# rikuu/Gap2Seq

Hardware: AMD Instinct MI355X
Metric: gaps filled/sec (whole node), k=31 synthetic 3 Mbp DBG (higher is better)
Workload: dtype u32

## Files before the change

### gap2seq_amd/csrc/d3_device.h

```cpp
#pragma once
#include <hip/hip_runtime_api.h>
#include <stdint.h>

#include "d2_device.h"
#include "fill_device.h"

#define G2S_D3_BLOCK_VARS 16u
#define G2S_RAND_BLOCK 4096u
#define G2S_RAND_WINDOW 160u
#define G2S_D3_TABLE_BUDGET (8u << 20)

#define G2S_D3_UNHANDLED 0x1u
#define G2S_D3_BUDGET 0x2u
#define G2S_D3_ANOMALY 0x4u

namespace g2s {

struct D3Gap {
  uint64_t arena_off;
  int32_t skip_thr;
  uint16_t lmf;
  uint8_t kind;
  uint8_t pad;
};
// ... 32 lines not shown
static_assert(sizeof(D3Var) == 64 && sizeof(D3Trace) == 32, "record layouts");

struct D3Summary {
  uint32_t status, unhandled, n_var, anomalies;
  unsigned long long host_items, host_segs, host_rnd;
  uint32_t handoff_waves, tiles;
  uint64_t table_entries, block_entries;
  uint64_t draws_min, draws_spread, draws_total;
  uint64_t xA, sA, xB, sB, xD, sD, segs, fill_bytes;
  uint32_t seg_gaps, filled;
  uint32_t rand_state[31];
  uint32_t trace_waves;
  uint32_t big_gaps;
  uint32_t traced_gaps;
  uint32_t spec_gaps;
};
static_assert(sizeof(D3Summary) <= 512, "the lap stamps live at byte 512 of the summary's slot");

struct RandTables {
  const uint32_t* hi = nullptr;
  const uint32_t* mid = nullptr;
  const uint32_t* lane = nullptr;
};
void rand_tables_host(uint32_t* hi , uint32_t* mid , uint32_t* lane );

struct D3Work {
  uint32_t* ginfo = nullptr;
  uint32_t* dmin = nullptr;
  uint32_t* dspread = nullptr;
  uint32_t* base = nullptr;
// ... 29 lines not shown
  int32_t k, skip_confident, all_paths, unique_paths;
  uint64_t max_states;
  uint64_t arena_base;
  uint32_t n;
  uint32_t has_skip;
  uint32_t seg_cap;
  uint32_t map_cap;
  uint32_t group_size;
  uint64_t sub_region;
  uint32_t laps;
  uint32_t self_clean;
  uint32_t base0, R0, d_in;
  const unsigned long long* d2_done;
  uint32_t d2_wgs;
  uint32_t restart;
};

hipError_t launch_rand_fill(hipStream_t st, uint32_t* rnd_all, const RandTables& rt, const D3Summary* sum_dev, uint64_t capacity,
                            uint64_t first_value = 0);

hipError_t launch_d3_sharded_classes(hipStream_t st, const D3Params& P, const D3Work& W, const GapOut* outs, const D3Gap* dgaps,
                                     bool summary_is_clean);
hipError_t launch_d3_sharded_tables(hipStream_t st, const D3Params& P, const D3Work& W, const GapOut* outs, const SubRec* sub,
                                    uint32_t* rnd_all, uint64_t rnd_capacity, uint32_t* group_fn );
hipError_t launch_d3_sharded_trace(hipStream_t st, const D3Params& P, const D3Work& W, const GapOut* outs, const SubRec* sub,
                                   const char* lastch_up, const char* lastch_dn, uint32_t* rnd_all, uint64_t rnd_capacity,
                                   void* results, char* arena, const D3Side& side, void* summary_host,
                                   hipEvent_t ev_d2 = nullptr );

hipError_t launch_rand_window(hipStream_t st, uint32_t* rnd_all, const uint32_t* link);
// ... 15 lines not shown
```

### gap2seq_amd/csrc/d3_device.hip

```cpp
#include "sync_debug.h"
#include <hip/hip_runtime.h>
#include <hip/hip_ext.h>

#include <algorithm>
#include <cstdlib>
#include <mutex>
#include <set>

#include "../../include/g2s.h"
#include "d3_device.h"
#include "envcache.hpp"

namespace {

using g2s::D3Gap;
using g2s::D3Params;
using g2s::D3Summary;
using g2s::D3Work;

__device__ __forceinline__ uint32_t uni(uint32_t x) { return (uint32_t)__builtin_amdgcn_readfirstlane((int)x); }

#define GI_CLASS(x) ((x) & 3u)
#define GI_FILLED 0x4u
#define GI_SKIPPED 0x8u
#define GI_BAD 0x10u
#define GI_MEM 0x20u
#define GI_PHASE_D 0x40u
#define D3_TILE 256u
#define GI_HOST 0x80u

__device__ __forceinline__ void stamp(const D3Work& W, int slot) {
  ((unsigned long long*)((char*)W.sum + 512))[slot] = wall_clock64();
}

__device__ __forceinline__ const SubRec* sub_of(const D3Params& P, const SubRec* sub, uint32_t i) {
  return sub + (uint64_t)(i / P.group_size) * P.sub_region;
}

__device__ __forceinline__ int gap_count(const GapOut& go, const D3Params& P, bool phase_d) {
  if (phase_d && !P.skip_confident && P.all_paths) return go.count_s;
  return go.c_count;
}

// ... 491 lines not shown
    const int d0 = (int)(s.depth_len & 0xFFFFu);
    if (d0 > len) break;
    if (s.flags & G2S_SUB_SOURCE) return 1 + len - d0;
    if (d0 == 0) break;
    const int nb = seg_nparents(s.par01, s.par23);
    const uint32_t at = (uint32_t)(1 + len - d0);
    if (nb == 0 || (nb > 1 && !(s.flags & G2S_SEG_ORDERED)) || (uint64_t)at >= avail || at >= nwin) break;
    const uint32_t rv = nb > 1 ? lwin[at] >> 1 : 0u;
    i = (int)seg_parent(s.par01, s.par23, nb == 1 ? 0 : pick_parent(rv, nb));
    if (i >= nsegs) break;
  }
  *bad = true;
  return 1;
}

#define D3_TAB_SEGS 512u
__global__ __launch_bounds__(256) void g2s_d3_tables(const D3Params P, const D3Work W, const SubRec* __restrict__ sub,
                                                     const uint32_t* __restrict__ rnd , uint64_t capacity) {
  __shared__ SegLite lseg[D3_TAB_SEGS];
  extern __shared__ __attribute__((aligned(16))) uint32_t lwin[];
  const uint32_t win_cap = P.map_cap + D3_TILE;
  const D3Summary* S = W.sum;
  const bool st0 = blockIdx.x == 0 && threadIdx.x == 0;
  if (st0) stamp(W, 3);
  const uint32_t status = S->status, tiles = S->tiles;
  const uint32_t tid = threadIdx.x;
  if (status) return;
  if (st0) stamp(W, 4);
  bool bad_any = false;
  for (uint32_t tile = blockIdx.x; tile < tiles; tile += gridDim.x) {
    const uint32_t v = W.tile_var[tile];
    const g2s::D3Var vd = W.vdesc[v];
    const uint32_t ns = vd.ns;
    const uint32_t d0 = (tile - vd.tile0) * D3_TILE, d = d0 + tid;
    const uint64_t at0 = (uint64_t)vd.base + d0;
    const bool mine = d <= vd.R;
    const uint32_t want = min(win_cap, min(vd.R - d0, D3_TILE - 1u) + vd.dmin + vd.dspread + 1u);
    if (st0) stamp(W, 5);
    __syncthreads();
    {
      const SegW* gs = (const SegW*)(sub + vd.sub_at);
      for (uint32_t q = tid; q < ns && q < D3_TAB_SEGS; q += 256u) {
        SegLite l;
        l.depth_len = gs[q].depth_len; l.par01 = gs[q].par01; l.par23 = gs[q].par23; l.flags = gs[q].flags;
        lseg[q] = l;
      }
      for (uint32_t x = tid; x < want; x += 256u) lwin[x] = at0 + x < capacity ? rnd[at0 + x] : 0u;
    }
    __syncthreads();
    if (st0) stamp(W, 6);
    if (mine) {
      bool bad = false;
      const uint64_t at = at0 + tid;
      const uint32_t nw = want > tid ? want - tid : 0u;
      const uint64_t av = capacity > at ? capacity - at : 0ull;
      const int draws = ns > D3_TAB_SEGS
                            ? d3_walk_count(vd.n_len, vd.len0, vd.len1, vd.start_seg, vd.start_t, (int)ns, (const SegW*)(sub + vd.sub_at), lwin + tid, nw, av, &bad)
                            : d3_walk_count_lite(vd.n_len, vd.len0, vd.len1, vd.start_seg, (int)ns, lseg, lwin + tid, nw, av, &bad);
      const int dev = draws - (int)vd.dmin;
      if (dev < 0 || dev > (int)vd.dspread) bad = true;
      W.tab[(uint64_t)vd.toff + d] = bad ? (uint16_t)0 : (uint16_t)dev;
      bad_any |= bad;
    }
  }
  if (bad_any) atomicAdd(&W.sum->anomalies, 1u);
  if (st0) stamp(W, 7);
  if (P.laps && tid == 0) {
    unsigned long long* laps = (unsigned long long*)((char*)W.sum + 512);
    if (blockIdx.x < tiles) atomicMax(&laps[32], wall_clock64());
    atomicMax(&laps[33], wall_clock64());
  }
}

__device__ __forceinline__ void d3_blocks_body(const D3Work& W, uint64_t first, uint64_t stride) {
  const D3Summary* S = W.sum;
  const uint32_t V = S->n_var;
  const uint32_t NB = (V + G2S_D3_BLOCK_VARS - 1u) / G2S_D3_BLOCK_VARS;
  const uint64_t TB = S->block_entries;
  for (uint64_t e = first; e < TB; e += stride) {
    uint32_t lo = 0, hi = NB;
    while (hi - lo > 1u) { const uint32_t mid = (lo + hi) >> 1; if ((uint64_t)W.blk_toff[mid] <= e) lo = mid; else hi = mid; }
    const uint32_t b = lo;
    uint32_t d = (uint32_t)(e - W.blk_toff[b]);
    const uint32_t v1 = min(V, (b + 1u) * G2S_D3_BLOCK_VARS);
    for (uint32_t v = b * G2S_D3_BLOCK_VARS; v < v1; v++) d += W.tab[(uint64_t)W.var_toff[v] + d];
    W.btab[e] = d;
  }
}
// ... 183 lines not shown
  (void)d3_classify_body(P, W, outs, dgaps, blockIdx.x * 256u + threadIdx.x, gridDim.x * 256u, nullptr, nullptr, nullptr, nullptr, red, false);
  (void)d3_handoff_body<true>(P, W, outs, sub, rnd, capacity, side, blockIdx.x * 256u + (threadIdx.x & ~63u), nullptr, nullptr, nullptr, nullptr);
  if ((threadIdx.x & 63u) == 0u) {
    asm volatile("s_waitcnt vmcnt(0)" ::: "memory");
    const unsigned int done = atomicAdd(&S->handoff_waves, 1u) + 1u;
    if (done == gridDim.x * 4u) {
      const unsigned long long items = atomicAdd(&S->host_items, 0ull);
      const uint32_t anomalies = atomicAdd(&S->anomalies, 0u), unhandled = atomicAdd(&S->unhandled, 0u);
      S->status = unhandled ? G2S_D3_UNHANDLED : 0u;
      __hip_atomic_store(side.count, (items & 0x7FFFFFFFFFFFFFFFull) | ((unsigned long long)((anomalies || unhandled) ? 1u : 0u) << 63),
                         __ATOMIC_RELEASE, __HIP_MEMORY_SCOPE_SYSTEM);
    }
  }
}
#define D3_BACK_TAB 24576u
__global__ __launch_bounds__(1024) void g2s_d3_back(const D3Params P, const D3Work W, const GapOut* __restrict__ outs,
                                                    const SubRec* __restrict__ sub, const uint32_t* __restrict__ Wd, uint64_t capacity,
                                                    const g2s::D3Side side) {
  __shared__ uint32_t total_dev;
  __shared__ unsigned long long lcur[3];
  if (threadIdx.x < 3u) lcur[threadIdx.x] = 0ull;
  __shared__ uint16_t ltab[D3_BACK_TAB];
  __shared__ uint32_t ltoff[1025], ldvar[1025];
  D3Summary* S = W.sum;
  if (threadIdx.x == 0) stamp(W, 8);
  const uint32_t status = S->status, V = S->n_var;
  const uint64_t T = S->table_entries;
  if (status) {
    if (threadIdx.x == 0) __hip_atomic_store(side.count, 1ull << 63, __ATOMIC_RELEASE, __HIP_MEMORY_SCOPE_SYSTEM);
    return;
  }
  const bool in_lds = T <= (uint64_t)D3_BACK_TAB && V <= 1024u;
  if (in_lds) {
    for (uint32_t e = threadIdx.x; e < (uint32_t)T; e += 1024u) ltab[e] = W.tab[e];
    if (threadIdx.x <= V) ltoff[threadIdx.x] = W.var_toff[threadIdx.x];
    __syncthreads();
    if (threadIdx.x == 0) {
      stamp(W, 9);
      uint32_t d = 0;
      for (uint32_t v = 0; v < V; v++) { ldvar[v] = d; d += ltab[ltoff[v] + d]; }
      ldvar[V] = d;
      total_dev = d;
    }
    __syncthreads();
    if (threadIdx.x <= V) W.dvar[threadIdx.x] = ldvar[threadIdx.x];
    const uint64_t total = S->draws_min + total_dev;
    if (threadIdx.x == 0) S->draws_total = total;
    if (threadIdx.x < 31u) {
      const uint32_t w = Wd[total + threadIdx.x];
      S->rand_state[threadIdx.x] = w;
      if (W.link) W.link[threadIdx.x] = w;
    }
  } else {
    d3_blocks_body(W, threadIdx.x, 1024u);
    __threadfence();
    __syncthreads();
    d3_chain_body(W, Wd, &total_dev);
    __threadfence();
    __syncthreads();
  }
  if (threadIdx.x == 0) stamp(W, 10);
  for (uint32_t i0 = (threadIdx.x >> 6) * 64u; i0 < P.n; i0 += 1024u)
    (void)d3_handoff_body<false>(P, W, outs, sub, Wd + 31, capacity, side, i0, in_lds ? ldvar : nullptr, in_lds ? ltab : nullptr,
                          in_lds ? ltoff : nullptr, lcur);
  __syncthreads();
  if (threadIdx.x == 0) {
    stamp(W, 11);
    const unsigned long long items = lcur[0];
    S->host_items = items; S->host_segs = lcur[1]; S->host_rnd = lcur[2];
    const uint32_t anomalies = atomicAdd(&S->anomalies, 0u);
    __hip_atomic_store(side.count, (items & 0x7FFFFFFFFFFFFFFFull) | ((unsigned long long)(anomalies ? 1u : 0u) << 63), __ATOMIC_RELEASE,
                       __HIP_MEMORY_SCOPE_SYSTEM);
    stamp(W, 12);
  }
}

template <int NW>
__global__ __launch_bounds__(64 * NW) void g2s_d3_trace(const D3Params P, const D3Work W, GapOut* __restrict__ outs,
                                                   const SubRec* __restrict__ sub, const char* __restrict__ chu,
                                                   const char* __restrict__ chd, const uint32_t* __restrict__ rnd,
                                                   uint64_t capacity, g2s_result* __restrict__ results,
                                                   char* __restrict__ arena, uint32_t* __restrict__ summary_host,
                                                   const g2s::D3Side side, uint32_t* __restrict__ clean_words ) {
  extern __shared__ __attribute__((aligned(16))) uint32_t lds[];
  D3Summary* S = W.sum;
  const uint32_t i = blockIdx.x;
  constexpr int NT = 64 * NW;
  const int tid = (int)threadIdx.x, lane = tid & 63;
  const bool w0 = tid < 64;
// ... 34 lines not shown
  if ((go.dflags & G2S_DEVA_D2_PENDING) && !(go.dflags & (G2S_DEVA_RUNS | G2S_DEVA_D2_FAILED)) && !P.skip_confident) {
    uint32_t v = go.dflags;
    for (uint32_t spin = 0; spin < (1u << 22) && !(v & (G2S_DEVA_RUNS | G2S_DEVA_D2_FAILED)); spin++) {
      __builtin_amdgcn_s_sleep(8);
      v = uni(__hip_atomic_load(&outs[i].dflags, __ATOMIC_ACQUIRE, __HIP_MEMORY_SCOPE_AGENT));
    }
    __builtin_amdgcn_fence(__ATOMIC_ACQUIRE, "agent");
    go.dflags = v;
    go.sub_vertices = uni(__hip_atomic_load(&outs[i].sub_vertices, __ATOMIC_RELAXED, __HIP_MEMORY_SCOPE_AGENT));
    go.sub_edges = uni(__hip_atomic_load(&outs[i].sub_edges, __ATOMIC_RELAXED, __HIP_MEMORY_SCOPE_AGENT));
    if (!(v & (G2S_DEVA_RUNS | G2S_DEVA_D2_FAILED))) d2_lost = true;
  }
  if ((go.dflags & G2S_DEVA_D2_PENDING) && (go.dflags & G2S_DEVA_D2_FAILED) && !(td.gi & GI_HOST) && (td.gi & GI_PHASE_D)) d2_lost = true;
  uint32_t gsp_all = 0, gsp_sent = 0;
  auto leave = [&](uint32_t fill_len) {
    if (!w0) return;
    uint32_t last = 0;
    if (lane == 0) {
      if (P.laps) {
        const unsigned long long tk4 = wall_clock64();
        atomicMax(&laps[14], tk1 ? tk1 - tk0 : 0ull); atomicMax(&laps[15], tk2 ? tk2 - tk1 : 0ull);
        atomicMax(&laps[16], tk3 ? tk3 - tk2 : 0ull); atomicMax(&laps[17], ((tk4 - tk0) << 24) | ((td.gi & GI_HOST) ? 1ull << 23 : 0ull) | (unsigned long long)(i & 0x7FFFFFu)); atomicMax(&laps[18], tk4);
        atomicMax(&laps[19], ((tk2 ? tk2 - tk1 : 0ull) << 32) | (hops << 16) | (tkm ? tkm - tk1 : 0ull));
        if ((P.laps >> 4) == i + 1u) { laps[26] = tk0; laps[27] = tk1; laps[28] = tkm; laps[29] = tk2; laps[30] = tk3; laps[31] = tk4; }
      }
      const uint32_t c = i & 63u, n = gridDim.x;
      const unsigned long long before = atomicAdd(&W.fill_bytes[c * 16u], (unsigned long long)fill_len | (1ull << 40));
      if (gsp_all) atomicAdd(&W.fill_bytes[c * 16u + 1u], (unsigned long long)gsp_all | ((unsigned long long)gsp_sent << 32));
      if ((uint32_t)(before >> 40) + 1u == (n + 63u - c) / 64u) last = atomicAdd(&S->trace_waves, 1u) + 1u == min(n, 64u) ? 1u : 0u;
    }
// ... 2 lines not shown
    if (P.d2_done && lane == 0)
      for (uint32_t spin = 0; spin < (1u << 22) && __hip_atomic_load(P.d2_done, __ATOMIC_ACQUIRE, __HIP_MEMORY_SCOPE_AGENT) < (unsigned long long)P.d2_wgs; spin++)
        __builtin_amdgcn_s_sleep(8);
    uint32_t* src = (uint32_t*)S;
    if (P.laps && lane == 0) laps[24] = wall_clock64();
    static_assert(sizeof(D3Summary) <= 512, "two words a lane");
    const uint32_t s0 = __hip_atomic_load(src + lane, __ATOMIC_RELAXED, __HIP_MEMORY_SCOPE_AGENT);
    const uint32_t s1 = __hip_atomic_load(src + 64 + lane, __ATOMIC_RELAXED, __HIP_MEMORY_SCOPE_AGENT);
    const unsigned long long* cl = (const unsigned long long*)(src + 256 + 32 * lane);
    const unsigned long long c0 = __hip_atomic_load(cl, __ATOMIC_RELAXED, __HIP_MEMORY_SCOPE_AGENT);
    const unsigned long long c1 = __hip_atomic_load(cl + 1, __ATOMIC_RELAXED, __HIP_MEMORY_SCOPE_AGENT);
    summary_host[lane] = s0;
    summary_host[64 + lane] = s1;
    ((unsigned long long*)(summary_host + 256 + 32 * lane))[0] = c0;
    ((unsigned long long*)(summary_host + 256 + 32 * lane))[1] = c1;
    if (P.self_clean) {
      src[lane] = 0u; src[64 + lane] = 0u;
      ((unsigned long long*)(src + 256 + 32 * lane))[0] = 0ull;
      ((unsigned long long*)(src + 256 + 32 * lane))[1] = 0ull;
    }
    if (P.self_clean && clean_words && lane < 32) clean_words[lane] = 0u;
    if (P.laps && lane == 0) { asm volatile("s_waitcnt vmcnt(0)" ::: "memory"); laps[25] = wall_clock64(); }
  };
  if (status) { leave(0u); return; }
  if (d2_lost) {
    if (tid == 0) { atomicAdd(&S->anomalies, 1u); arena[td.arena_off + td.lmf] = '\0'; }
    asm volatile("s_waitcnt vmcnt(0)" ::: "memory");
    leave(0u);
    return;
  }
// ... 470 lines not shown
  if (P.n == 0) return hipSuccess;
  hipError_t e = summary_is_clean ? hipSuccess : hipMemsetAsync(W.sum, 0, 1024 + 64 * 128, st);
  if (e != hipSuccess) return e;
  hipLaunchKernelGGL(g2s_d3_classify, dim3((P.n + 255u) / 256u), dim3(256), 0, st, P, W, outs, dgaps);
  launch_scan(st, P, W, outs);
  return hipGetLastError();
}
hipError_t launch_d3_sharded_tables(hipStream_t st, const D3Params& P, const D3Work& W, const GapOut* outs, const SubRec* sub,
                                    uint32_t* rnd_all, uint64_t rnd_capacity, uint32_t* group_fn) {
  if (P.n == 0) return hipSuccess;
  launch_scan(st, P, W, outs);
  const uint32_t tgrid = std::min(8192u, std::max(128u, P.n / 2u));
  const size_t win = ((size_t)P.map_cap + 256) * 4;
  hipError_t e = hipFuncSetAttribute((const void*)g2s_d3_tables, hipFuncAttributeMaxDynamicSharedMemorySize, (int)win);
  if (e != hipSuccess) return e;
  hipLaunchKernelGGL(g2s_d3_tables, dim3(tgrid), dim3(256), win, st, P, W, sub, rnd_all + 31, rnd_capacity);
  hipLaunchKernelGGL(g2s_d3_blocks, dim3(256), dim3(256), 0, st, W);
  hipLaunchKernelGGL(g2s_d3_groupfn, dim3(std::min(256u, (P.R0 + 256u) / 256u)), dim3(256), 0, st, W, P.R0, group_fn);
  return hipGetLastError();
}
hipError_t launch_d3_sharded_trace(hipStream_t st, const D3Params& P, const D3Work& W, const GapOut* outs, const SubRec* sub,
                                   const char* lastch_up, const char* lastch_dn, uint32_t* rnd_all, uint64_t rnd_capacity,
                                   void* results, char* arena, const D3Side& side, void* summary_host, hipEvent_t ev_d2) {
  if (P.n == 0) return hipSuccess;
  hipLaunchKernelGGL(g2s_d3_chain, dim3(1), dim3(1024), 0, st, W, rnd_all, P.base0, P.d_in);
  if (ev_d2) { const hipError_t e2 = hipStreamWaitEvent(st, ev_d2, 0); if (e2 != hipSuccess) return e2; }
  hipLaunchKernelGGL(g2s_d3_handoff, dim3((P.n + 63u) / 64u), dim3(64), 0, st, P, W, outs, sub, rnd_all + 31, rnd_capacity, side);
  const size_t lds = (size_t)P.seg_cap * (sizeof(SegRec) + 16) + (size_t)P.map_cap * 8 + 16;
  hipError_t e = hipFuncSetAttribute((const void*)g2s_d3_trace<1>, hipFuncAttributeMaxDynamicSharedMemorySize, (int)lds);
  if (e != hipSuccess) return e;
  hipLaunchKernelGGL(g2s_d3_trace<1>, dim3(P.n), dim3(64), lds, st, P, W, const_cast<GapOut*>(outs), sub, lastch_up, lastch_dn, rnd_all + 31, rnd_capacity,
// ... 10 lines not shown
  (void)gaps;
  (void)rt;
  static_assert(sizeof(D3Summary) <= 1024, "summary slot");
  hipError_t e = summary_is_clean ? hipSuccess : hipMemsetAsync(W.sum, 0, 1024 + 64 * 128, st);
  if (e != hipSuccess) return e;
  const bool short_list = P.n <= D3_FRONT_GAPS;
  if (P.restart) {
    if (ev_d2) { e = hipStreamWaitEvent(st, ev_d2, 0); if (e != hipSuccess) return e; }
    hipLaunchKernelGGL(g2s_d3_restart, dim3((P.n + 255u) / 256u), dim3(256), 0, st, P, W, outs, dgaps, sub, rnd_all + 31, rnd_capacity, side);
  } else if (short_list) hipLaunchKernelGGL(g2s_d3_front, dim3(1), dim3(1024), 0, st, P, W, outs, dgaps);
  else {
    hipLaunchKernelGGL(g2s_d3_classify, dim3((P.n + 255u) / 256u), dim3(256), 0, st, P, W, outs, dgaps);
    launch_scan(st, P, W, outs);
  }
  const uint32_t tgrid = std::min(8192u, std::max(128u, P.n / 2u));
  const size_t win = ((size_t)P.map_cap + 256) * 4;
  if (!P.restart) {
    e = hipFuncSetAttribute((const void*)g2s_d3_tables, hipFuncAttributeMaxDynamicSharedMemorySize, (int)win);
    if (e != hipSuccess) return e;
    hipLaunchKernelGGL(g2s_d3_tables, dim3(tgrid), dim3(256), win, st, P, W, sub, rnd_all + 31, rnd_capacity);
  }
  if (ev_d2 && short_list && !P.restart) { e = hipStreamWaitEvent(st, ev_d2, 0); if (e != hipSuccess) return e; }
  if (P.restart) (void)ev_chain;
  else if (short_list) {
    hipLaunchKernelGGL(g2s_d3_back, dim3(1), dim3(1024), 0, st, P, W, outs, sub, rnd_all, rnd_capacity, side);
    if (ev_chain) { e = hipEventRecord(ev_chain, st); if (e != hipSuccess) return e; }
  } else {
    hipLaunchKernelGGL(g2s_d3_blocks, dim3(256), dim3(256), 0, st, W);
    hipLaunchKernelGGL(g2s_d3_chain, dim3(1), dim3(1024), 0, st, W, rnd_all, 0u, 0u);
    if (ev_chain) { e = hipEventRecord(ev_chain, st); if (e != hipSuccess) return e; }
    if (ev_d2) { e = hipStreamWaitEvent(st, ev_d2, 0); if (e != hipSuccess) return e; }
    hipLaunchKernelGGL(g2s_d3_handoff, dim3((P.n + 63u) / 64u), dim3(64), 0, st, P, W, outs, sub, rnd_all + 31, rnd_capacity, side);
  }
  const size_t lds = (size_t)P.seg_cap * (sizeof(SegRec) + 16) + (size_t)P.map_cap * 8 + 16;
  const char* waves_s = GENV("G2S_TRACE_WAVES");
  const int waves_env = waves_s ? atoi(waves_s) : 0;
  const bool four = waves_env ? waves_env == 4 : P.n <= 768u;
  e = hipFuncSetAttribute(four ? (const void*)g2s_d3_trace<4> : (const void*)g2s_d3_trace<1>, hipFuncAttributeMaxDynamicSharedMemorySize, (int)lds);
  if (e != hipSuccess) return e;
  if (ev_stop != nullptr) {
// ... 19 lines not shown
```

### gap2seq_amd/csrc/g2s_api.hip

```cpp
#include <hip/hip_runtime.h>
#include <cstdarg>
#include <sys/prctl.h>
#include <pthread.h>
#include <sched.h>
#include <time.h>

#include <algorithm>
#include <atomic>
#include <chrono>
#include <cstdio>
#include <cstdlib>
#include <condition_variable>
#include <cstring>
#include <functional>
#include <mutex>
#include <string>
#include <thread>
#include <vector>

#include "../../include/g2s.h"
#include "../../include/g2s_test.h"
#include "envcache.hpp"
#include "d2_device.h"
#include "d3_device.h"
// ... 681 lines not shown
  int team_sessions = 1;
  int peer_asked_for = -1;
  bool self_cleaned = false;
  std::vector<uint32_t> host_order;
  size_t side_dirty = SIZE_MAX;
  size_t side_layout_n = 0;
  uint32_t timed_seq = 0;
  std::chrono::steady_clock::time_point lap_fill_queued, lap_d3_queued, lap_handed, lap_finished, lap_synced, lap_end;
  bool laps_valid = false;
  int resident_strikes = 0;
  int segw_quiet = 0;
  hipEvent_t ev_segw = nullptr;
  g2s_session* twins[G2S_MAX_IN_FLIGHT - 1] = {};
  DevBuf d_link;
  hipEvent_t ev_chain = nullptr;
  void* d3_pending = nullptr;
  struct InFlight { g2s_batch* b = nullptr; g2s_session* on = nullptr; g2s_result* results = nullptr; char* arena = nullptr; size_t cap = 0;
                    const g2s_gap* gaps = nullptr; size_t n = 0; double ms_prepare = 0;
                    bool d3_queued = false;
                    bool chained = false; };
  InFlight inflight[G2S_MAX_IN_FLIGHT];
  int n_inflight = 0;
  int internal_calls = 0;
  uint64_t begun = 0;
  g2s_batch* share_batch = nullptr;
  int share_step = 0;
  bool share_timed = false, share_two = false;
  uint32_t share_win[G2S_RAND_WINDOW];
  bool resident_off = false;
  uint32_t seed0 = 0;
// ... 2304 lines not shown
  bool discard = false;
  D3Side side_h;
  D3Work W;
  D3Summary* hsum = nullptr;
  hipEvent_t d3_begin = nullptr;
  g2s_result* results = nullptr;
  char* arena = nullptr;
  std::chrono::steady_clock::time_point t_enter, t_launched;
  bool sharded = false;
  D3Params P;
  D3Side side_dev;
  void* res_dev = nullptr;
  char* arena_dev = nullptr;
  const D3Gap* dgaps_dev = nullptr;
  void* summary_dev = nullptr;
  uint32_t* group_fn = nullptr;
  uint32_t* group_fn_dev = nullptr;
  size_t rnd_cap = 0;
};
static int resident_d3_launch(g2s_session* s, const ResidentList& L, bool timed, bool rand_launched, g2s_result* results, char* arena,
                              bool no_spin, bool sharded = false ,
                              g2s_session* chain_from = nullptr ) {
  const size_t n = L.n;
  const Graph& g = *s->graph->g;
  const FillParams fp = fill_params_of(s);
  const auto t_enter = std::chrono::steady_clock::now();
  if (n > 20480 || L.dmax > 12000 || rand_capacity(L.rnd_cap) >= (1ull << 31)) return 1;
  if (hipSetDevice(s->device) != hipSuccess) return fail(G2S_ERR_NO_DEVICE, "cannot select device");
  D3Summary* hsum = (D3Summary*)((char*)L.pin->p + n * sizeof(D3Gap) + 16 - (n * sizeof(D3Gap)) % 16);
  const size_t rnd_cap = rand_capacity(L.rnd_cap);
  HIP_TRY_S(s->d_d3.ensure(d3_work_bytes((uint32_t)n)));
  D3Side side, side_h;
  {
    side_h.cap_items = n;
    const bool deep = L.dmax >= 2500;
    side_h.cap_segs = deep ? std::min<uint64_t>((uint64_t)n * 4096u, 4ull << 20) + 65536u : std::max<uint64_t>((uint64_t)n * 16u, 65536u);
    const size_t side_rnd = std::max(rnd_cap, rand_capacity(L.rnd_sum));
// ... 61 lines not shown
  memset(&P, 0, sizeof P);
  P.k = fp.k; P.skip_confident = fp.skip_confident ? 1 : 0; P.all_paths = fp.all_paths ? 1 : 0; P.unique_paths = fp.unique_paths ? 1 : 0;
  P.max_states = (uint64_t)std::max<int64_t>(s->params.max_mem, 1 << 16) / 64;
  P.n = (uint32_t)n;
  P.has_skip = L.has_skip ? 1u : 0u;
  P.arena_base = 0;
  P.group_size = (uint32_t)std::max<size_t>(L.group_size, 1);
  P.sub_region = L.sub_region;
  P.laps = GENV("G2S_DEBUG") ? (1u | (GENV("G2S_DEBUG_GAP") ? ((uint32_t)atoi(GENV("G2S_DEBUG_GAP")) + 1u) << 4 : 0u)) : 0u;
  const bool self_clean = L.groups.size() == 1 && L.outs_dev == (const GapOut*)s->d_outs.p && !P.laps && !sharded;
  P.self_clean = self_clean ? 1u : 0u;
  if (W.d2out) { P.d2_done = (const unsigned long long*)s->d_counter.p + 9; P.d2_wgs = s->d2_wgs; }
  P.seg_cap = fp.skip_confident ? G2S_SEG_CAP : 192u;
  P.map_cap = ((uint32_t)L.dmax + 2u + 3u) & ~3u;
  P.restart = L.restart ? 1u : 0u;
  if (sharded) {
    HIP_TRY_S(launch_d3_sharded_classes(st, P, W, L.outs_dev, (const D3Gap*)d_dgaps, s->d_d3.clean >= 1024 + 64 * 128));
    HIP_TRY_S(hipMemcpyAsync(hsum, W.sum, sizeof(D3Summary), hipMemcpyDeviceToHost, st));
  } else
  HIP_TRY_S(launch_d3(st, P, W, L.gaps_dev, L.outs_dev, dgap_on_device ? (const D3Gap*)s->d_dgap.p : (const D3Gap*)d_dgaps, L.sub_dev,
                    (const char*)s->d_lastch.p, (const char*)s->d_lastch.p + g.n, s->rtab, (uint32_t*)s->d_rnd.p,
                    (uint64_t)rnd_cap, res_dev, (char*)arena_dev, side, (char*)d_dgaps + ((char*)hsum - (char*)L.pin->p),
                    s->d_d3.clean >= 1024 + 64 * 128, self_clean ? (uint32_t*)s->d_counter.p : nullptr,
                    no_spin ? s->ev_chain : nullptr ,
                    (W.d2out && (s->d2_wait || L.restart)) ? s->ev_d2 : nullptr,
                    timed ? s->ev[3] : nullptr ));
  s->d_d3.clean = 0;
  {
    D3Pending* dp = new D3Pending;
    dp->L = L; dp->timed = timed; dp->res_direct = res_direct; dp->arena_direct = arena_direct;
    dp->self_clean = self_clean; dp->side_h = side_h; dp->W = W; dp->hsum = hsum; dp->d3_begin = d3_begin; dp->results = results;
    dp->arena = arena; dp->t_enter = t_enter; dp->t_launched = std::chrono::steady_clock::now();
    dp->sharded = sharded; dp->P = P; dp->side_dev = side; dp->res_dev = res_dev; dp->arena_dev = (char*)arena_dev;
    dp->dgaps_dev = (const D3Gap*)d_dgaps; dp->summary_dev = (char*)d_dgaps + ((char*)hsum - (char*)L.pin->p);
    delete (D3Pending*)s->d3_pending;
    s->d3_pending = dp;
  }
  return G2S_OK;
}
static int resident_d3_sharded_tables(g2s_session* s, uint32_t base0, uint32_t R0, const uint32_t* win) {
  D3Pending* dp = (D3Pending*)s->d3_pending;
  if (!dp || !dp->sharded) return fail(G2S_ERR_ARG, "sharded list: no group pending");
  if (hipSetDevice(s->device) != hipSuccess) return fail(G2S_ERR_NO_DEVICE, "cannot select device");
  const size_t n = dp->L.n;
  const size_t rnd_cap = rand_capacity((size_t)base0 + (size_t)R0 + dp->L.rnd_cap);
  dp->rnd_cap = rnd_cap;
  {
    char* hsum_c = (char*)dp->hsum;
    uint32_t* hwin = (uint32_t*)(hsum_c + 1024 + 64 * 128);
// ... 173 lines not shown
    for (size_t x = 0; x < ni; x++) host_fill_bytes += (uint64_t)rs_host[side_h.items[x].gap].fill_len;
    if (const char* path = GENV("G2S_HOST_ITEMS_DUMP")) {
      if (FILE* f = fopen(path, "wb")) {
        for (size_t x = 0; x < ni; x++) {
          const D3HostItem& h = side_h.items[x];
          const GapOut& go = side_h.outs[x];
          const int32_t hd[8] = {(int32_t)h.gap, (int32_t)h.n_segs, go.c_count, go.n_len, go.len[0], go.len[1], go.reached_j, go.final_d};
          fwrite(hd, sizeof hd, 1, f);
          fwrite(side_h.segs + h.seg_off, sizeof(SegRec), h.n_segs, f);
        }
        fclose(f);
      }
    }
  }
  const auto t_finished = std::chrono::steady_clock::now();
  HIP_TRY_S(hipStreamSynchronize(st));
  const auto t_synced = std::chrono::steady_clock::now();
  float ms_d3 = 0;
  if (timed) HIP_TRY_S(hipEventElapsedTime(&ms_d3, d3_begin, s->ev[3]));
  *ms_d3_out = ms_d3;
  if (GENV("G2S_DEBUG")) {
    unsigned long long lp[34];
    HIP_TRY_S(hipMemcpy(lp, (char*)W.sum + 512, sizeof lp, hipMemcpyDeviceToHost));
    auto us = [&](int a, int b) { return lp[a] && lp[b] ? ((double)lp[b] - (double)lp[a]) / 100.0 : -1.0; };
    fprintf(stderr, "[g2s] phase D3 laps (us): front classify %.1f scan %.1f | to tables %.1f: status %.1f records %.1f closure %.1f walks %.1f | to back %.1f: tables into LDS %.1f chain %.1f hand-off %.1f fence %.1f | to trace %.1f, longest wave: to closure %.1f walk %.1f bases %.1f all %.1f, first entry to last end %.1f\n",
            us(0, 1), us(1, 2), us(2, 3), us(3, 4), us(4, 5), us(5, 6), us(6, 7), us(7, 8), us(8, 9), us(9, 10), us(10, 11), us(11, 12), us(12, 13),
            lp[14] / 100.0, lp[15] / 100.0, lp[16] / 100.0, (double)(lp[17] >> 24) / 100.0, us(13, 18));
    fprintf(stderr, "[g2s] the longest wave of the trace kernel: gap %llu%s\n", lp[17] & 0x7FFFFFull, (lp[17] >> 23) & 1ull ? " (handed to the host)" : "");
    fprintf(stderr, "[g2s] scan (us): sums %.1f, base + layout pass %.1f, table offsets + records %.1f\n", us(20, 21), us(21, 22), us(22, 23));
    fprintf(stderr, "[g2s] the last wave of the trace kernel: the summary's copy to the host begins %.1f us after the kernel's first entry and takes %.1f us\n", us(13, 24), us(24, 25));
    if (GENV("G2S_DEBUG_GAP") && lp[26])
// ... 164 lines not shown
    rand_launched = true;
  }
  if (b->pre_launched) {
    rl = b->pre;
    b->pre_launched = false;
  } else {
    const int rc = resident_launch_fill(b, &rl, results, arena);
    if (rc != G2S_OK) {
      if (rand_launched) (void)hipStreamSynchronize(s->stream2);
      return rc;
    }
  }
  ResidentList L = resident_list_of(b, b->arena_base, b->arena_base + b->arena_bytes);
  L.rnd_sum = b->rnd_sum; L.restart = b->set_list;
  if (b->arena_base) { shift_arena_offsets(s, n, b->arena_base); s->desc_owner = nullptr; }
  return resident_d3_launch(s, L, rl.timed, rand_launched, results, arena, no_spin, false, chain_from);
}
static int run_resident_finish(g2s_batch* b, const ResidentLaunch& rl, std::chrono::steady_clock::time_point t_enter) {
  g2s_session* s = b->s;
  const size_t n = b->jobs.size();
  double ms_d3 = 0;
  bool fell_back = false;
  const int rc = resident_d3_wait(s, &b->timing, &ms_d3, &fell_back);
  if (rc != G2S_OK) return rc;
  if (s->self_cleaned) { s->d_outs.clean = n * sizeof(GapOut); s->d_counter.clean = 128; }
  else { const int r2 = resident_reset_fill(s, n); if (r2 != G2S_OK) return r2; }
  s->self_cleaned = false;
  if (fell_back) { b->timing.resident_fallbacks++; return 1; }
  float ms_fill = 0, ms_segw = 0;
  if (rl.timed) HIP_TRY(hipEventElapsedTime(&ms_fill, s->ev[1], s->ev[2]));
  if (rl.timed && rl.segw) HIP_TRY(hipEventElapsedTime(&ms_segw, s->ev[2], s->ev_segw));
// ... 1198 lines not shown
```

Before: 3.043 million.

## Fold D3 back pass into last tables workgroup and poll host done flag

The single-workgroup back kernel is turned into a templated body. On the short-list path the last workgroup of g2s_d3_tables runs it, detected with an atomic counter, which removes one kernel launch and its dependency gap. The trace kernel also writes a system-scope sequence number into pinned host memory after the summary copy, so the host can spin on that flag instead of calling hipStreamSynchronize. In exchange it adds extra system fences in the trace leave path, a 256-thread back body with smaller LDS tables, and a host busy-wait.

```diff
diff --git a/gap2seq_amd/csrc/d3_device.h b/gap2seq_amd/csrc/d3_device.h
--- a/gap2seq_amd/csrc/d3_device.h
+++ b/gap2seq_amd/csrc/d3_device.h
@@ -70,6 +70,7 @@
   uint32_t big_gaps;
   uint32_t traced_gaps;
   uint32_t spec_gaps;
+  uint32_t tables_wgs;
 };
 static_assert(sizeof(D3Summary) <= 512, "the lap stamps live at byte 512 of the summary's slot");
 
@@ -129,6 +130,7 @@
   const unsigned long long* d2_done;
   uint32_t d2_wgs;
   uint32_t restart;
+  uint32_t done_seq;
 };
 
 hipError_t launch_rand_fill(hipStream_t st, uint32_t* rnd_all, const RandTables& rt, const D3Summary* sum_dev, uint64_t capacity,
diff --git a/gap2seq_amd/csrc/d3_device.hip b/gap2seq_amd/csrc/d3_device.hip
--- a/gap2seq_amd/csrc/d3_device.hip
+++ b/gap2seq_amd/csrc/d3_device.hip
@@ -27,6 +27,7 @@
 #define GI_MEM 0x20u
 #define GI_PHASE_D 0x40u
 #define D3_TILE 256u
+#define D3_TAB_SEGS 512u
 #define GI_HOST 0x80u
 
 __device__ __forceinline__ void stamp(const D3Work& W, int slot) {
@@ -548,64 +549,6 @@
   return 1;
 }
 
-#define D3_TAB_SEGS 512u
-__global__ __launch_bounds__(256) void g2s_d3_tables(const D3Params P, const D3Work W, const SubRec* __restrict__ sub,
-                                                     const uint32_t* __restrict__ rnd , uint64_t capacity) {
-  __shared__ SegLite lseg[D3_TAB_SEGS];
-  extern __shared__ __attribute__((aligned(16))) uint32_t lwin[];
-  const uint32_t win_cap = P.map_cap + D3_TILE;
-  const D3Summary* S = W.sum;
-  const bool st0 = blockIdx.x == 0 && threadIdx.x == 0;
-  if (st0) stamp(W, 3);
-  const uint32_t status = S->status, tiles = S->tiles;
-  const uint32_t tid = threadIdx.x;
-  if (status) return;
-  if (st0) stamp(W, 4);
-  bool bad_any = false;
-  for (uint32_t tile = blockIdx.x; tile < tiles; tile += gridDim.x) {
-    const uint32_t v = W.tile_var[tile];
-    const g2s::D3Var vd = W.vdesc[v];
-    const uint32_t ns = vd.ns;
-    const uint32_t d0 = (tile - vd.tile0) * D3_TILE, d = d0 + tid;
-    const uint64_t at0 = (uint64_t)vd.base + d0;
-    const bool mine = d <= vd.R;
-    const uint32_t want = min(win_cap, min(vd.R - d0, D3_TILE - 1u) + vd.dmin + vd.dspread + 1u);
-    if (st0) stamp(W, 5);
-    __syncthreads();
-    {
-      const SegW* gs = (const SegW*)(sub + vd.sub_at);
-      for (uint32_t q = tid; q < ns && q < D3_TAB_SEGS; q += 256u) {
-        SegLite l;
-        l.depth_len = gs[q].depth_len; l.par01 = gs[q].par01; l.par23 = gs[q].par23; l.flags = gs[q].flags;
-        lseg[q] = l;
-      }
-      for (uint32_t x = tid; x < want; x += 256u) lwin[x] = at0 + x < capacity ? rnd[at0 + x] : 0u;
-    }
-    __syncthreads();
-    if (st0) stamp(W, 6);
-    if (mine) {
-      bool bad = false;
-      const uint64_t at = at0 + tid;
-      const uint32_t nw = want > tid ? want - tid : 0u;
-      const uint64_t av = capacity > at ? capacity - at : 0ull;
-      const int draws = ns > D3_TAB_SEGS
-                            ? d3_walk_count(vd.n_len, vd.len0, vd.len1, vd.start_seg, vd.start_t, (int)ns, (const SegW*)(sub + vd.sub_at), lwin + tid, nw, av, &bad)
-                            : d3_walk_count_lite(vd.n_len, vd.len0, vd.len1, vd.start_seg, (int)ns, lseg, lwin + tid, nw, av, &bad);
-      const int dev = draws - (int)vd.dmin;
-      if (dev < 0 || dev > (int)vd.dspread) bad = true;
-      W.tab[(uint64_t)vd.toff + d] = bad ? (uint16_t)0 : (uint16_t)dev;
-      bad_any |= bad;
-    }
-  }
-  if (bad_any) atomicAdd(&W.sum->anomalies, 1u);
-  if (st0) stamp(W, 7);
-  if (P.laps && tid == 0) {
-    unsigned long long* laps = (unsigned long long*)((char*)W.sum + 512);
-    if (blockIdx.x < tiles) atomicMax(&laps[32], wall_clock64());
-    atomicMax(&laps[33], wall_clock64());
-  }
-}
-
 __device__ __forceinline__ void d3_blocks_body(const D3Work& W, uint64_t first, uint64_t stride) {
   const D3Summary* S = W.sum;
   const uint32_t V = S->n_var;
@@ -819,37 +762,34 @@
   }
 }
 #define D3_BACK_TAB 24576u
-__global__ __launch_bounds__(1024) void g2s_d3_back(const D3Params P, const D3Work W, const GapOut* __restrict__ outs,
-                                                    const SubRec* __restrict__ sub, const uint32_t* __restrict__ Wd, uint64_t capacity,
-                                                    const g2s::D3Side side) {
-  __shared__ uint32_t total_dev;
-  __shared__ unsigned long long lcur[3];
+template <uint32_t NT>
+__device__ __forceinline__ void d3_back_body(const D3Params& P, const D3Work& W, const GapOut* __restrict__ outs,
+                                             const SubRec* __restrict__ sub, const uint32_t* __restrict__ Wd, uint64_t capacity,
+                                             const g2s::D3Side& side, uint32_t status, uint32_t V, uint64_t T, uint16_t* ltab,
+                                             uint32_t tab_cap, uint32_t* ltoff, uint32_t* ldvar, uint32_t var_cap,
+                                             unsigned long long* lcur, uint32_t* total_dev) {
+  D3Summary* S = W.sum;
   if (threadIdx.x < 3u) lcur[threadIdx.x] = 0ull;
-  __shared__ uint16_t ltab[D3_BACK_TAB];
-  __shared__ uint32_t ltoff[1025], ldvar[1025];
-  D3Summary* S = W.sum;
   if (threadIdx.x == 0) stamp(W, 8);
-  const uint32_t status = S->status, V = S->n_var;
-  const uint64_t T = S->table_entries;
   if (status) {
     if (threadIdx.x == 0) __hip_atomic_store(side.count, 1ull << 63, __ATOMIC_RELEASE, __HIP_MEMORY_SCOPE_SYSTEM);
     return;
   }
-  const bool in_lds = T <= (uint64_t)D3_BACK_TAB && V <= 1024u;
+  const bool in_lds = T <= (uint64_t)tab_cap && V <= var_cap;
   if (in_lds) {
-    for (uint32_t e = threadIdx.x; e < (uint32_t)T; e += 1024u) ltab[e] = W.tab[e];
-    if (threadIdx.x <= V) ltoff[threadIdx.x] = W.var_toff[threadIdx.x];
+    for (uint32_t e = threadIdx.x; e < (uint32_t)T; e += NT) ltab[e] = W.tab[e];
+    for (uint32_t v = threadIdx.x; v <= V; v += NT) ltoff[v] = W.var_toff[v];
     __syncthreads();
     if (threadIdx.x == 0) {
       stamp(W, 9);
       uint32_t d = 0;
       for (uint32_t v = 0; v < V; v++) { ldvar[v] = d; d += ltab[ltoff[v] + d]; }
       ldvar[V] = d;
-      total_dev = d;
+      *total_dev = d;
     }
     __syncthreads();
-    if (threadIdx.x <= V) W.dvar[threadIdx.x] = ldvar[threadIdx.x];
-    const uint64_t total = S->draws_min + total_dev;
+    for (uint32_t v = threadIdx.x; v <= V; v += NT) W.dvar[v] = ldvar[v];
+    const uint64_t total = S->draws_min + *total_dev;
     if (threadIdx.x == 0) S->draws_total = total;
     if (threadIdx.x < 31u) {
       const uint32_t w = Wd[total + threadIdx.x];
@@ -857,15 +797,15 @@
       if (W.link) W.link[threadIdx.x] = w;
     }
   } else {
-    d3_blocks_body(W, threadIdx.x, 1024u);
+    d3_blocks_body(W, threadIdx.x, NT);
     __threadfence();
     __syncthreads();
-    d3_chain_body(W, Wd, &total_dev);
+    d3_chain_body(W, Wd, total_dev);
     __threadfence();
     __syncthreads();
   }
   if (threadIdx.x == 0) stamp(W, 10);
-  for (uint32_t i0 = (threadIdx.x >> 6) * 64u; i0 < P.n; i0 += 1024u)
+  for (uint32_t i0 = (threadIdx.x >> 6) * 64u; i0 < P.n; i0 += NT)
     (void)d3_handoff_body<false>(P, W, outs, sub, Wd + 31, capacity, side, i0, in_lds ? ldvar : nullptr, in_lds ? ltab : nullptr,
                           in_lds ? ltoff : nullptr, lcur);
   __syncthreads();
@@ -878,6 +818,99 @@
                        __HIP_MEMORY_SCOPE_SYSTEM);
     stamp(W, 12);
   }
+}
+__global__ __launch_bounds__(1024) void g2s_d3_back(const D3Params P, const D3Work W, const GapOut* __restrict__ outs,
+                                                    const SubRec* __restrict__ sub, const uint32_t* __restrict__ Wd, uint64_t capacity,
+                                                    const g2s::D3Side side) {
+  __shared__ uint32_t total_dev;
+  __shared__ unsigned long long lcur[3];
+  __shared__ uint16_t ltab[D3_BACK_TAB];
+  __shared__ uint32_t ltoff[1025], ldvar[1025];
+  const D3Summary* S = W.sum;
+  const uint32_t status = S->status, V = S->n_var;
+  const uint64_t T = S->table_entries;
+  d3_back_body<1024u>(P, W, outs, sub, Wd, capacity, side, status, V, T, ltab, D3_BACK_TAB, ltoff, ldvar, 1024u, lcur, &total_dev);
+}
+
+#define D3_FOLD_VARS 511u
+#define D3_FOLD_TAB 8192u
+#define D3_FOLD_LDS(tab) (32u + 2u * 4u * (D3_FOLD_VARS + 1u) + 2u * (tab))
+__global__ __launch_bounds__(256) void g2s_d3_tables(const D3Params P, const D3Work W, const SubRec* __restrict__ sub,
+                                                     const uint32_t* __restrict__ rnd , uint64_t capacity,
+                                                     const GapOut* __restrict__ outs, const g2s::D3Side side, int32_t fold_tab) {
+  __shared__ SegLite lseg[D3_TAB_SEGS];
+  __shared__ uint32_t last_wg;
+  extern __shared__ __attribute__((aligned(16))) uint32_t lwin[];
+  const uint32_t win_cap = P.map_cap + D3_TILE;
+  const D3Summary* S = W.sum;
+  const bool st0 = blockIdx.x == 0 && threadIdx.x == 0;
+  if (st0) stamp(W, 3);
+  const uint32_t status = S->status, tiles = S->tiles, n_var = S->n_var;
+  const uint64_t table_entries = S->table_entries;
+  const uint32_t tid = threadIdx.x;
+  const bool fold = fold_tab >= 0;
+  if (status && !fold) return;
+  if (st0) stamp(W, 4);
+  bool bad_any = false;
+  for (uint32_t tile = blockIdx.x; tile < (status ? 0u : tiles); tile += gridDim.x) {
+    const uint32_t v = W.tile_var[tile];
+    const g2s::D3Var vd = W.vdesc[v];
+    const uint32_t ns = vd.ns;
+    const uint32_t d0 = (tile - vd.tile0) * D3_TILE, d = d0 + tid;
+    const uint64_t at0 = (uint64_t)vd.base + d0;
+    const bool mine = d <= vd.R;
+    const uint32_t want = min(win_cap, min(vd.R - d0, D3_TILE - 1u) + vd.dmin + vd.dspread + 1u);
+    if (st0) stamp(W, 5);
+    __syncthreads();
+    {
+      const SegW* gs = (const SegW*)(sub + vd.sub_at);
+      for (uint32_t q = tid; q < ns && q < D3_TAB_SEGS; q += 256u) {
+        SegLite l;
+        l.depth_len = gs[q].depth_len; l.par01 = gs[q].par01; l.par23 = gs[q].par23; l.flags = gs[q].flags;
+        lseg[q] = l;
+      }
+      for (uint32_t x = tid; x < want; x += 256u) lwin[x] = at0 + x < capacity ? rnd[at0 + x] : 0u;
+    }
+    __syncthreads();
+    if (st0) stamp(W, 6);
+    if (mine) {
+      bool bad = false;
+      const uint64_t at = at0 + tid;
+      const uint32_t nw = want > tid ? want - tid : 0u;
+      const uint64_t av = capacity > at ? capacity - at : 0ull;
+      const int draws = ns > D3_TAB_SEGS
+                            ? d3_walk_count(vd.n_len, vd.len0, vd.len1, vd.start_seg, vd.start_t, (int)ns, (const SegW*)(sub + vd.sub_at), lwin + tid, nw, av, &bad)
+                            : d3_walk_count_lite(vd.n_len, vd.len0, vd.len1, vd.start_seg, (int)ns, lseg, lwin + tid, nw, av, &bad);
+      const int dev = draws - (int)vd.dmin;
+      if (dev < 0 || dev > (int)vd.dspread) bad = true;
+      W.tab[(uint64_t)vd.toff + d] = bad ? (uint16_t)0 : (uint16_t)dev;
+      bad_any |= bad;
+    }
+  }
+  if (bad_any) atomicAdd(&W.sum->anomalies, 1u);
+  if (st0) stamp(W, 7);
+  if (P.laps && tid == 0) {
+    unsigned long long* laps = (unsigned long long*)((char*)W.sum + 512);
+    if (blockIdx.x < tiles) atomicMax(&laps[32], wall_clock64());
+    atomicMax(&laps[33], wall_clock64());
+  }
+  if (!fold) return;
+  __threadfence();
+  __syncthreads();
+  if (tid == 0) {
+#ifdef G2S_SYNC_DEBUG
+    g2s_sync_jitter(0xD4u);
+    g2s_wait_all();
+#endif
+    last_wg = atomicAdd(&W.sum->tables_wgs, 1u) + 1u == gridDim.x ? 1u : 0u;
+  }
+  __syncthreads();
+  if (!last_wg) return;
+  __builtin_amdgcn_fence(__ATOMIC_ACQUIRE, "agent");
+  unsigned long long* lcur = (unsigned long long*)lwin;
+  uint32_t* ltoff = lwin + 8, *ldvar = ltoff + (D3_FOLD_VARS + 1u);
+  d3_back_body<256u>(P, W, outs, sub, rnd - 31, capacity, side, status, n_var, table_entries, (uint16_t*)(ldvar + (D3_FOLD_VARS + 1u)),
+                     (uint32_t)fold_tab, ltoff, ldvar, D3_FOLD_VARS, lcur, lwin + 6);
 }
 
 template <int NW>
@@ -942,6 +975,10 @@
   if ((go.dflags & G2S_DEVA_D2_PENDING) && (go.dflags & G2S_DEVA_D2_FAILED) && !(td.gi & GI_HOST) && (td.gi & GI_PHASE_D)) d2_lost = true;
   uint32_t gsp_all = 0, gsp_sent = 0;
   auto leave = [&](uint32_t fill_len) {
+    if (P.done_seq) {
+      __threadfence_system();
+      if constexpr (NW > 1) __syncthreads();
+    }
     if (!w0) return;
     uint32_t last = 0;
     if (lane == 0) {
@@ -974,6 +1011,10 @@
     summary_host[64 + lane] = s1;
     ((unsigned long long*)(summary_host + 256 + 32 * lane))[0] = c0;
     ((unsigned long long*)(summary_host + 256 + 32 * lane))[1] = c1;
+    if (P.done_seq) {
+      __threadfence_system();
+      if (lane == 0) __hip_atomic_store(summary_host + 128, P.done_seq, __ATOMIC_RELEASE, __HIP_MEMORY_SCOPE_SYSTEM);
+    }
     if (P.self_clean) {
       src[lane] = 0u; src[64 + lane] = 0u;
       ((unsigned long long*)(src + 256 + 32 * lane))[0] = 0ull;
@@ -1474,7 +1515,7 @@
   const size_t win = ((size_t)P.map_cap + 256) * 4;
   hipError_t e = hipFuncSetAttribute((const void*)g2s_d3_tables, hipFuncAttributeMaxDynamicSharedMemorySize, (int)win);
   if (e != hipSuccess) return e;
-  hipLaunchKernelGGL(g2s_d3_tables, dim3(tgrid), dim3(256), win, st, P, W, sub, rnd_all + 31, rnd_capacity);
+  hipLaunchKernelGGL(g2s_d3_tables, dim3(tgrid), dim3(256), win, st, P, W, sub, rnd_all + 31, rnd_capacity, outs, D3Side(), -1);
   hipLaunchKernelGGL(g2s_d3_blocks, dim3(256), dim3(256), 0, st, W);
   hipLaunchKernelGGL(g2s_d3_groupfn, dim3(std::min(256u, (P.R0 + 256u) / 256u)), dim3(256), 0, st, W, P.R0, group_fn);
   return hipGetLastError();
@@ -1515,16 +1556,24 @@
     launch_scan(st, P, W, outs);
   }
   const uint32_t tgrid = std::min(8192u, std::max(128u, P.n / 2u));
-  const size_t win = ((size_t)P.map_cap + 256) * 4;
+  size_t win = ((size_t)P.map_cap + 256) * 4;
+  bool fold = short_list && !P.restart && !ev_d2;
+  int32_t fold_tab = -1;
+  if (fold) { const char* bl = GENV("G2S_D3_BACK_LAUNCH"); if (bl && atoi(bl) != 0) fold = false; }
+  if (fold) {
+    const char* ft = GENV("G2S_D3_FOLD_TAB");
+    fold_tab = ft ? std::max(0, std::min(atoi(ft), (int)D3_FOLD_TAB)) : (int32_t)D3_FOLD_TAB;
+    win = std::max(win, (size_t)D3_FOLD_LDS((uint32_t)fold_tab));
+  }
   if (!P.restart) {
     e = hipFuncSetAttribute((const void*)g2s_d3_tables, hipFuncAttributeMaxDynamicSharedMemorySize, (int)win);
     if (e != hipSuccess) return e;
-    hipLaunchKernelGGL(g2s_d3_tables, dim3(tgrid), dim3(256), win, st, P, W, sub, rnd_all + 31, rnd_capacity);
+    hipLaunchKernelGGL(g2s_d3_tables, dim3(tgrid), dim3(256), win, st, P, W, sub, rnd_all + 31, rnd_capacity, outs, side, fold_tab);
   }
   if (ev_d2 && short_list && !P.restart) { e = hipStreamWaitEvent(st, ev_d2, 0); if (e != hipSuccess) return e; }
   if (P.restart) (void)ev_chain;
   else if (short_list) {
-    hipLaunchKernelGGL(g2s_d3_back, dim3(1), dim3(1024), 0, st, P, W, outs, sub, rnd_all, rnd_capacity, side);
+    if (!fold) hipLaunchKernelGGL(g2s_d3_back, dim3(1), dim3(1024), 0, st, P, W, outs, sub, rnd_all, rnd_capacity, side);
     if (ev_chain) { e = hipEventRecord(ev_chain, st); if (e != hipSuccess) return e; }
   } else {
     hipLaunchKernelGGL(g2s_d3_blocks, dim3(256), dim3(256), 0, st, W);
diff --git a/gap2seq_amd/csrc/g2s_api.hip b/gap2seq_amd/csrc/g2s_api.hip
--- a/gap2seq_amd/csrc/g2s_api.hip
+++ b/gap2seq_amd/csrc/g2s_api.hip
@@ -719,6 +719,7 @@
   g2s_session* twins[G2S_MAX_IN_FLIGHT - 1] = {};
   DevBuf d_link;
   hipEvent_t ev_chain = nullptr;
+  uint32_t d3_seq = 0;
   void* d3_pending = nullptr;
   struct InFlight { g2s_batch* b = nullptr; g2s_session* on = nullptr; g2s_result* results = nullptr; char* arena = nullptr; size_t cap = 0;
                     const g2s_gap* gaps = nullptr; size_t n = 0; double ms_prepare = 0;
@@ -3053,13 +3054,15 @@
   char* arena_dev = nullptr;
   const D3Gap* dgaps_dev = nullptr;
   void* summary_dev = nullptr;
+  uint32_t done_seq = 0;
   uint32_t* group_fn = nullptr;
   uint32_t* group_fn_dev = nullptr;
   size_t rnd_cap = 0;
 };
 static int resident_d3_launch(g2s_session* s, const ResidentList& L, bool timed, bool rand_launched, g2s_result* results, char* arena,
                               bool no_spin, bool sharded = false ,
-                              g2s_session* chain_from = nullptr ) {
+                              g2s_session* chain_from = nullptr ,
+                              bool poll_done = false ) {
   const size_t n = L.n;
   const Graph& g = *s->graph->g;
   const FillParams fp = fill_params_of(s);
@@ -3151,6 +3154,14 @@
   P.seg_cap = fp.skip_confident ? G2S_SEG_CAP : 192u;
   P.map_cap = ((uint32_t)L.dmax + 2u + 3u) & ~3u;
   P.restart = L.restart ? 1u : 0u;
+  if (poll_done && self_clean && !timed && !no_spin) {
+    const char* sy = GENV("G2S_D3_SYNC");
+    if (!(sy && atoi(sy) != 0)) {
+      if (++s->d3_seq == 0u) s->d3_seq = 1u;
+      P.done_seq = s->d3_seq;
+      __atomic_store_n((uint32_t*)hsum + 128, 0u, __ATOMIC_RELAXED);
+    }
+  }
   if (sharded) {
     HIP_TRY_S(launch_d3_sharded_classes(st, P, W, L.outs_dev, (const D3Gap*)d_dgaps, s->d_d3.clean >= 1024 + 64 * 128));
     HIP_TRY_S(hipMemcpyAsync(hsum, W.sum, sizeof(D3Summary), hipMemcpyDeviceToHost, st));
@@ -3170,6 +3181,7 @@
     dp->arena = arena; dp->t_enter = t_enter; dp->t_launched = std::chrono::steady_clock::now();
     dp->sharded = sharded; dp->P = P; dp->side_dev = side; dp->res_dev = res_dev; dp->arena_dev = (char*)arena_dev;
     dp->dgaps_dev = (const D3Gap*)d_dgaps; dp->summary_dev = (char*)d_dgaps + ((char*)hsum - (char*)L.pin->p);
+    dp->done_seq = P.done_seq;
     delete (D3Pending*)s->d3_pending;
     s->d3_pending = dp;
   }
@@ -3373,7 +3385,16 @@
     }
   }
   const auto t_finished = std::chrono::steady_clock::now();
-  HIP_TRY_S(hipStreamSynchronize(st));
+  bool done_seen = false;
+  if (dpp->done_seq) {
+    const uint32_t* done = (const uint32_t*)hsum + 128;
+    for (unsigned spins = 0;; spins++) {
+      if (__atomic_load_n(done, __ATOMIC_ACQUIRE) == dpp->done_seq) { done_seen = true; break; }
+      if ((spins & 1023u) == 1023u && hipStreamQuery(st) != hipErrorNotReady) break;
+      cpu_relax();
+    }
+  }
+  if (!done_seen) HIP_TRY_S(hipStreamSynchronize(st));
   const auto t_synced = std::chrono::steady_clock::now();
   float ms_d3 = 0;
   if (timed) HIP_TRY_S(hipEventElapsedTime(&ms_d3, d3_begin, s->ev[3]));
@@ -3568,7 +3589,7 @@
   ResidentList L = resident_list_of(b, b->arena_base, b->arena_base + b->arena_bytes);
   L.rnd_sum = b->rnd_sum; L.restart = b->set_list;
   if (b->arena_base) { shift_arena_offsets(s, n, b->arena_base); s->desc_owner = nullptr; }
-  return resident_d3_launch(s, L, rl.timed, rand_launched, results, arena, no_spin, false, chain_from);
+  return resident_d3_launch(s, L, rl.timed, rand_launched, results, arena, no_spin, false, chain_from, !no_spin);
 }
 static int run_resident_finish(g2s_batch* b, const ResidentLaunch& rl, std::chrono::steady_clock::time_point t_enter) {
   g2s_session* s = b->s;
```

Result: slower. 2.609 million (-14.2%).
